# rizar/attention-lvcsr

Hardware: AMD Instinct MI355X
Metric: encoder+attention+decoder training frames/sec (whole node) (higher is better)
Workload: dtype f32; 1 GPU; wsj_base: B=16 utterances x T=800 frames x F=40 fbank per GPU, L=100 labels; 256x256x256x256 BiGRU subsample [1, 1, 2, 2], content_and_conv attention, 256-unit GRU decoder; global_batch=16, per_gpu_batch=16, ragged=False, parallelism=dp1, optimizer=clip100+adadelta+maxnorm1, hip_graph=True, priming_steps=2, encoder_kernels=persistent clusters, full=False

## Files before the change

attention-lvcsr_amd/csrc/gemm.hip:

```cpp
#include "common.h"
#include "lvsr_hip.h"
#include "graph_cache.h"

#define BM 64
#define BN 64
#define BK 16
#define LDS_LD (BM + 4)

struct GemmArgs {
    const float* A; const float* B; float* C; const float* bias;
    int M, N, K, lda, ldb, ldc, transA, transB;
    float alpha, beta;
    int ksplit;
    int kchunk;
    float* part;
    int batch;
    long long sA, sB, sC;
};

__global__ __launch_bounds__(256) void lvsr_sgemm_kernel(GemmArgs g) {
    __shared__ float As[BK][LDS_LD];
    __shared__ float Bs[BK][LDS_LD];
    const int tid = threadIdx.x, lane = tid & 63, wave = tid >> 6;
    const int m0 = blockIdx.y * BM, n0 = blockIdx.x * BN;
    int zsplit = blockIdx.z;
    if (g.batch > 1) {
        g.A += blockIdx.z * g.sA; g.B += blockIdx.z * g.sB; g.C += blockIdx.z * g.sC;
        zsplit = 0;
    }
    const int kbeg = zsplit * g.kchunk;
    const int kend = min(g.K, kbeg + g.kchunk);
    const int rowbase = (wave >> 1) * 32, colbase = (wave & 1) * 32;
    f32x4 acc[2][2];
#pragma unroll
    for (int i = 0; i < 2; ++i)
#pragma unroll
        for (int j = 0; j < 2; ++j) acc[i][j] = (f32x4){0.f, 0.f, 0.f, 0.f};

    for (int k0 = kbeg; k0 < kend; k0 += BK) {
        if (!g.transA) {
            const int kk = tid & 15, mm = tid >> 4;
#pragma unroll
            for (int p = 0; p < 4; ++p) {
                const int m = m0 + mm + p * 16, k = k0 + kk;
                As[kk][mm + p * 16] = (m < g.M && k < kend) ? g.A[(size_t)m * g.lda + k] : 0.f;
            }
        } else {
            const int mm = tid & 63, kk = tid >> 6;
#pragma unroll
            for (int p = 0; p < 4; ++p) {
                const int m = m0 + mm, k = k0 + kk + p * 4;
                As[kk + p * 4][mm] = (m < g.M && k < kend) ? g.A[(size_t)k * g.lda + m] : 0.f;
            }
        }
        if (!g.transB) {
            const int nn = tid & 63, kk = tid >> 6;
#pragma unroll
            for (int p = 0; p < 4; ++p) {
                const int n = n0 + nn, k = k0 + kk + p * 4;
                Bs[kk + p * 4][nn] = (n < g.N && k < kend) ? g.B[(size_t)k * g.ldb + n] : 0.f;
            }
        } else {
            const int kk = tid & 15, nn = tid >> 4;
#pragma unroll
            for (int p = 0; p < 4; ++p) {
                const int n = n0 + nn + p * 16, k = k0 + kk;
                Bs[kk][nn + p * 16] = (n < g.N && k < kend) ? g.B[(size_t)n * g.ldb + k] : 0.f;
            }
        }
        __syncthreads();
#pragma unroll
        for (int ks = 0; ks < BK; ks += 4) {
            const int kr = ks + (lane >> 4), li = lane & 15;
            float a[2], b[2];
            a[0] = As[kr][rowbase + li];
            a[1] = As[kr][rowbase + 16 + li];
            b[0] = Bs[kr][colbase + li];
            b[1] = Bs[kr][colbase + 16 + li];
#pragma unroll
            for (int i = 0; i < 2; ++i)
#pragma unroll
                for (int j = 0; j < 2; ++j)
                    acc[i][j] = __builtin_amdgcn_mfma_f32_16x16x4f32(a[i], b[j], acc[i][j], 0, 0, 0);
        }
        __syncthreads();
// ... 254 lines not shown
        if (more) {
            if (inside && k0 + 2 * GK <= kend) {
                gemm1_tile_load_fast<!TA, TM>(g.A, g.lda, m0, k0 + GK, ra);
                gemm1_tile_load_fast<TB, TN>(g.B, g.ldb, n0, k0 + GK, rb);
            } else {
                gemm1_tile_load<!TA, TM>(g.A, g.lda, m0, g.M, k0 + GK, kend, vecA, ra);
                gemm1_tile_load<TB, TN>(g.B, g.ldb, n0, g.N, k0 + GK, kend, vecB, rb);
            }
        }
        const int kr0 = lane >> 5, li = lane & 31;
        float pa[2][MI], pb[2][NI];
#pragma unroll
        for (int i = 0; i < MI; ++i) pa[0][i] = As[cur][kr0][wm + 32 * i + li];
#pragma unroll
        for (int j = 0; j < NI; ++j) pb[0][j] = Bs[cur][kr0][wn + 32 * j + li];
#pragma unroll
        for (int s = 0; s < GK / 2; ++s) {
            const int c = s & 1, n = c ^ 1;
            if (s + 1 < GK / 2) {
                const int kr = 2 * (s + 1) + kr0;
#pragma unroll
                for (int i = 0; i < MI; ++i) pa[n][i] = As[cur][kr][wm + 32 * i + li];
#pragma unroll
                for (int j = 0; j < NI; ++j) pb[n][j] = Bs[cur][kr][wn + 32 * j + li];
            }
            __builtin_amdgcn_sched_barrier(0);
#pragma unroll
            for (int i = 0; i < MI; ++i)
#pragma unroll
                for (int j = 0; j < NI; ++j)
                    acc[i][j] = __builtin_amdgcn_mfma_f32_32x32x2f32(pa[c][i], pb[c][j], acc[i][j], 0, 0, 0);
            __builtin_amdgcn_sched_barrier(0);
        }
        if (more) {
            gemm1_tile_store<!TA, TM>(As[cur ^ 1], ra);
            gemm1_tile_store<TB, TN>(Bs[cur ^ 1], rb);
        }
        __syncthreads();
        cur ^= 1;
    }
#pragma unroll
    for (int i = 0; i < MI; ++i)
#pragma unroll
        for (int j = 0; j < NI; ++j)
#pragma unroll
            for (int r = 0; r < 16; ++r) {
                const int m = m0 + wm + i * 32 + (r & 3) + 8 * (r >> 2) + 4 * (lane >> 5);
                const int n = n0 + wn + j * 32 + (lane & 31);
                if (m < g.M && n < g.N) {
                    if (g.ksplit > 1) {
                        g.part[((size_t)bz * g.M + m) * g.N + n] = acc[i][j][r];
                    } else {
                        float v = g.alpha * acc[i][j][r];
                        if (g.beta != 0.f) v += g.beta * g.C[(size_t)m * g.ldc + n];
                        if (g.bias) v += g.bias[n];
                        g.C[(size_t)m * g.ldc + n] = v;
                    }
                }
            }
}
template <bool TA, bool TB, bool FAST>
__device__ __forceinline__ void sgemm128_tile(GemmArgs g, int bx, int by, int bz) { sgemm_tile<128, 128, TA, TB, FAST>(g, bx, by, bz); }

template <bool TA, bool TB, bool FAST>
__global__ __launch_bounds__(256) void lvsr_sgemm64_kernel(GemmArgs g) {
    const int total = gridDim.x * gridDim.y * gridDim.z;
    const int t = gemm_xcd_order(blockIdx.x + gridDim.x * (blockIdx.y + gridDim.y * blockIdx.z), total);
    sgemm_tile_kmajor<64, 64, TA, TB, FAST>(g, t % gridDim.x, (t / gridDim.x) % gridDim.y, t / (gridDim.x * gridDim.y));
}

template <bool TA, bool TB, bool FAST>
__global__ __launch_bounds__(256) void lvsr_sgemm128_kernel(GemmArgs g) {
    const int total = gridDim.x * gridDim.y * gridDim.z;
    const int t = gemm_xcd_order(blockIdx.x + gridDim.x * (blockIdx.y + gridDim.y * blockIdx.z), total);
    sgemm128_tile<TA, TB, FAST>(g, t % gridDim.x, (t / gridDim.x) % gridDim.y, t / (gridDim.x * gridDim.y));
}

#define GROUP_MAX 40
struct GroupDesc {
    const float* A; const float* B; float* C;
    int M, N, K, lda, ldb, ldc;
    float beta;
    int ksplit, kchunk, gx, gy, unit0;
    long long part_off;
};
struct GroupPack { GroupDesc d[GROUP_MAX]; int n, total; float* part; };

template <bool FAST>
__global__ __launch_bounds__(256) void lvsr_sgemm128_grouped_tn_kernel(GroupPack pk) {
    const int t = gemm_xcd_order(blockIdx.x, pk.total);
    int p = 0;
    for (int x = 1; x < pk.n; ++x)
        if (t >= pk.d[x].unit0) p = x;
    const GroupDesc& d = pk.d[p];
    const int local = t - d.unit0;
    GemmArgs g;
    g.A = d.A; g.B = d.B; g.C = d.C; g.bias = nullptr;
    g.M = d.M; g.N = d.N; g.K = d.K; g.lda = d.lda; g.ldb = d.ldb; g.ldc = d.ldc; g.transA = 1; g.transB = 0;
    g.alpha = 1.f; g.beta = d.beta; g.ksplit = d.ksplit; g.kchunk = d.kchunk; g.part = pk.part + d.part_off;
    g.batch = 1; g.sA = g.sB = g.sC = 0;
    sgemm128_tile<true, false, FAST>(g, local % d.gx, (local / d.gx) % d.gy, local / (d.gx * d.gy));
}

__global__ __launch_bounds__(256) void lvsr_sgemm_grouped_reduce(GroupPack pk) {
    const GroupDesc& d = pk.d[blockIdx.y];
    if (d.ksplit <= 1) return;
    const size_t total = (size_t)d.M * d.N;
    const float* part = pk.part + d.part_off;
    for (size_t idx = (size_t)blockIdx.x * 256 + threadIdx.x; idx < total; idx += (size_t)gridDim.x * 256) {
        const int m = (int)(idx / d.N), n = (int)(idx % d.N);
        float s = 0.f;
        for (int z = 0; z < d.ksplit; ++z) s += part[(size_t)z * total + idx];
        if (d.beta != 0.f) s += d.beta * d.C[(size_t)m * d.ldc + n];
        d.C[(size_t)m * d.ldc + n] = s;
    }
}

__global__ __launch_bounds__(256) void lvsr_sgemm_splitk_reduce(GemmArgs g) {
    const size_t total = (size_t)g.M * g.N;
    for (size_t idx = (size_t)blockIdx.x * blockDim.x + threadIdx.x; idx < total; idx += (size_t)gridDim.x * blockDim.x) {
        const int m = (int)(idx / g.N), n = (int)(idx % g.N);
        float s = 0.f;
        for (int z = 0; z < g.ksplit; ++z) s += g.part[(size_t)z * total + idx];
        float v = g.alpha * s;
        if (g.beta != 0.f) v += g.beta * g.C[(size_t)m * g.ldc + n];
        if (g.bias) v += g.bias[n];
        g.C[(size_t)m * g.ldc + n] = v;
    }
}

__global__ __launch_bounds__(256) void lvsr_colsum_kernel(const float* X, int M, int N, int ldx, float* out, float beta,
                                                          int rows_per, float* part) {
    __shared__ float red[4][64];
    const int n = blockIdx.x * 64 + (threadIdx.x & 63);
    const int g = threadIdx.x >> 6;
    const int m0 = blockIdx.y * rows_per, m1 = min(M, m0 + rows_per);
    float s0 = 0.f, s1 = 0.f, s2 = 0.f, s3 = 0.f;
    if (n < N) {
        int m = m0 + g;
        for (; m + 12 < m1; m += 16) {
            s0 += X[(size_t)m * ldx + n];
            s1 += X[(size_t)(m + 4) * ldx + n];
            s2 += X[(size_t)(m + 8) * ldx + n];
            s3 += X[(size_t)(m + 12) * ldx + n];
        }
        for (; m < m1; m += 4) s0 += X[(size_t)m * ldx + n];
    }
    red[g][threadIdx.x & 63] = (s0 + s1) + (s2 + s3);
    __syncthreads();
    if (g == 0 && n < N) {
        const int c = threadIdx.x & 63;
        const float v = ((red[0][c] + red[1][c]) + red[2][c]) + red[3][c];
        if (part) part[(size_t)blockIdx.y * N + n] = v;
        else out[n] = (beta != 0.f ? beta * out[n] : 0.f) + v;
    }
}

#define COLSUM_MANY_MAX 32
struct ColsumMember { const float* X; float* out; float* part; int M, N, ldx, S, rows_per, nx, block0, fin0; float beta; };
struct ColsumPack { ColsumMember m[COLSUM_MANY_MAX]; int n; };
__global__ __launch_bounds__(256) void lvsr_colsum_many_kernel(ColsumPack pk) {
    __shared__ float red[4][64];
    int p = 0;
    for (int i = 1; i < pk.n; ++i)
        if ((int)blockIdx.x >= pk.m[i].block0) p = i;
    const ColsumMember& c = pk.m[p];
    const int local = blockIdx.x - c.block0, bx = local % c.nx, by = local / c.nx;
    const int n = bx * 64 + (threadIdx.x & 63);
    const int g = threadIdx.x >> 6;
    const int m0 = by * c.rows_per, m1 = min(c.M, m0 + c.rows_per);
    const float* X = c.X;
    const int ldx = c.ldx;
    float s0 = 0.f, s1 = 0.f, s2 = 0.f, s3 = 0.f;
    if (n < c.N) {
        int m = m0 + g;
        for (; m + 12 < m1; m += 16) {
            s0 += X[(size_t)m * ldx + n];
            s1 += X[(size_t)(m + 4) * ldx + n];
            s2 += X[(size_t)(m + 8) * ldx + n];
            s3 += X[(size_t)(m + 12) * ldx + n];
        }
        for (; m < m1; m += 4) s0 += X[(size_t)m * ldx + n];
    }
    red[g][threadIdx.x & 63] = (s0 + s1) + (s2 + s3);
    __syncthreads();
    if (g == 0 && n < c.N) {
        const int col = threadIdx.x & 63;
        const float v = ((red[0][col] + red[1][col]) + red[2][col]) + red[3][col];
        if (c.S > 1) c.part[(size_t)by * c.N + n] = v;
        else c.out[n] = (c.beta != 0.f ? c.beta * c.out[n] : 0.f) + v;
    }
}
__global__ __launch_bounds__(256) void lvsr_colsum_many_finish(ColsumPack pk) {
    int p = 0;
    for (int i = 1; i < pk.n; ++i)
        if ((int)blockIdx.x >= pk.m[i].fin0) p = i;
    const ColsumMember& c = pk.m[p];
// ... 73 lines not shown
    if (M == 0 || N == 0) return LVSR_OK;
    GemmArgs g;
    g.batch = batch; g.sA = sA; g.sB = sB; g.sC = sC;
    if (batch > 1) ws = nullptr;
    g.A = A; g.B = B; g.C = C; g.bias = bias;
    g.M = M; g.N = N; g.K = K; g.lda = lda; g.ldb = ldb; g.ldc = ldc; g.transA = transA; g.transB = transB;
    g.alpha = alpha; g.beta = beta; g.ksplit = 1; g.kchunk = 0; g.part = nullptr;
    const bool big = (M >= 96 && N >= 96) || (min(M, N) >= 32 && max(M, N) >= 256 && K >= 2048);
    int tm = big ? GM : BM, tn = big ? GN : BN;
    const int tk = big ? GK : BK;
    int tiles = ((M + tm - 1) / tm) * ((N + tn - 1) / tn);
    const int mid_max = lvsr_knob(LVSR_KNOB_GEMM_MID_TILES) > 0 ? lvsr_knob(LVSR_KNOB_GEMM_MID_TILES) : 2048;
    const bool mid = big && batch == 1 && (tiles < 256 || (tiles < mid_max && K <= 2048));
    if (mid) { tm = 64; tn = 64; tiles = ((M + 63) / 64) * ((N + 63) / 64); }
    g.kchunk = ((K + tk - 1) / tk) * tk;
    if (g.kchunk == 0) g.kchunk = tk;
    const int slots = mid ? 1024 : 512;
    if (ws && 2 * tiles <= slots && K >= 1024) {
        int want = (slots + tiles - 1) / tiles;
        int maxk = K / 256;
        if (want > maxk) want = maxk;
        long long need = (long long)want * M * N * 4;
        while (want > 1 && need > ws_bytes) { --want; need = (long long)want * M * N * 4; }
        if (want > 1) {
            int chunk = (K + want - 1) / want;
            chunk = ((chunk + tk - 1) / tk) * tk;
            g.ksplit = (K + chunk - 1) / chunk;
            g.kchunk = chunk;
            g.part = ws;
        }
    }
    dim3 grid((N + tn - 1) / tn, (M + tm - 1) / tm, batch > 1 ? batch : g.ksplit);
    hipStream_t st = (hipStream_t)stream;
    if (!big) {
        hipLaunchKernelGGL(lvsr_sgemm_kernel, grid, dim3(256), 0, st, g);
    } else {
        const bool fast = (lda & 3) == 0 && (ldb & 3) == 0 && (((size_t)A) & 15) == 0 && (((size_t)B) & 15) == 0 &&
                          (batch == 1 || ((sA & 3) == 0 && (sB & 3) == 0));
#define LVSR_GEMM128(TA_, TB_)                                                                              \
    do {                                                                                                    \
        if (fast) hipLaunchKernelGGL((lvsr_sgemm128_kernel<TA_, TB_, true>), grid, dim3(256), 0, st, g);    \
        else hipLaunchKernelGGL((lvsr_sgemm128_kernel<TA_, TB_, false>), grid, dim3(256), 0, st, g);        \
    } while (0)
#define LVSR_GEMM64(TA_, TB_)                                                                               \
    do {                                                                                                    \
        if (fast) hipLaunchKernelGGL((lvsr_sgemm64_kernel<TA_, TB_, true>), grid, dim3(256), 0, st, g);     \
        else hipLaunchKernelGGL((lvsr_sgemm64_kernel<TA_, TB_, false>), grid, dim3(256), 0, st, g);         \
    } while (0)
        if (mid) {
            if (!transA && !transB) LVSR_GEMM64(false, false);
            else if (transA && !transB) LVSR_GEMM64(true, false);
            else if (!transA && transB) LVSR_GEMM64(false, true);
            else LVSR_GEMM64(true, true);
        } else if (!transA && !transB) LVSR_GEMM128(false, false);
        else if (transA && !transB) LVSR_GEMM128(true, false);
        else if (!transA && transB) LVSR_GEMM128(false, true);
        else LVSR_GEMM128(true, true);
#undef LVSR_GEMM128
#undef LVSR_GEMM64
    }
    if (g.ksplit > 1) {
        int nb = (int)(((size_t)M * N + 255) / 256);
        if (nb > 2048) nb = 2048;
        hipLaunchKernelGGL(lvsr_sgemm_splitk_reduce, dim3(nb), dim3(256), 0, st, g);
    }
    return lvsr_check_launch("lvsr_sgemm");
}

int lvsr_sgemm(void* stream, int transA, int transB, int M, int N, int K, float alpha, const float* A, int lda,
               const float* B, int ldb, float beta, float* C, int ldc, const float* bias, float* ws,
               long long ws_bytes) {
    return sgemm_launch(stream, transA, transB, M, N, K, alpha, A, lda, B, ldb, beta, C, ldc, bias, ws, ws_bytes, 1, 0, 0, 0);
}

int lvsr_sgemm_batched(void* stream, int transA, int transB, int M, int N, int K, float alpha, const float* A, int lda,
                       long long strideA, const float* B, int ldb, long long strideB, float beta, float* C, int ldc,
                       long long strideC, int batch) {
    LVSR_REQUIRE(batch >= 0, "lvsr_sgemm_batched: negative batch");
    if (batch == 0) return LVSR_OK;
    return sgemm_launch(stream, transA, transB, M, N, K, alpha, A, lda, B, ldb, beta, C, ldc, nullptr, nullptr, 0, batch,
                        strideA, strideB, strideC);
}

int lvsr_sgemm_tn_grouped(void* stream, const lvsr_gemm_desc* descs, int n, float* ws, long long ws_bytes) {
    LVSR_REQUIRE(n >= 0 && (n == 0 || descs), "lvsr_sgemm_tn_grouped: bad arguments");
    hipStream_t st = (hipStream_t)stream;
    for (int i = 0; i < n; ++i)
        LVSR_REQUIRE(descs[i].A && descs[i].B && descs[i].C && descs[i].M > 0 && descs[i].N > 0 && descs[i].K > 0,
                     "lvsr_sgemm_tn_grouped: bad descriptor %d", i);
    auto aligned = [](const lvsr_gemm_desc& s) {
        return (s.lda & 3) == 0 && (s.ldb & 3) == 0 && (((size_t)s.A) & 15) == 0 && (((size_t)s.B) & 15) == 0;
    };
    int target = 1024;
    if (ws) {
        for (;; target += 512) {
            long long need = 0;
            bool splits = false;
            for (int i = 0; i < n; ++i) {
                const int want = (descs[i].K + target - 1) / target;
                if (want > 1) { need += (long long)want * descs[i].M * descs[i].N; splits = true; }
            }
            if (!splits || need * 4 <= ws_bytes) break;
        }
    }
    long long off = 0;
    for (int pass = 0; pass < 2; ++pass) {
        GroupPack pk;
        pk.n = 0; pk.part = ws;
        int units = 0;
        bool any_split = false;
        auto launch = [&]() {
            if (pk.n == 0) return;
            pk.total = units;
            if (pass == 0) hipLaunchKernelGGL(lvsr_sgemm128_grouped_tn_kernel<true>, dim3(units), dim3(256), 0, st, pk);
            else hipLaunchKernelGGL(lvsr_sgemm128_grouped_tn_kernel<false>, dim3(units), dim3(256), 0, st, pk);
            if (any_split) hipLaunchKernelGGL(lvsr_sgemm_grouped_reduce, dim3(32, pk.n), dim3(256), 0, st, pk);
            pk.n = 0; units = 0; any_split = false;
        };
        for (int i = 0; i < n; ++i) {
            const lvsr_gemm_desc& s = descs[i];
            if (aligned(s) != (pass == 0)) continue;
            if (pk.n == GROUP_MAX) launch();
            GroupDesc& d = pk.d[pk.n++];
            d.A = s.A; d.B = s.B; d.C = s.C; d.M = s.M; d.N = s.N; d.K = s.K; d.lda = s.lda; d.ldb = s.ldb; d.ldc = s.ldc; d.beta = s.beta;
            d.gx = (s.N + GN - 1) / GN; d.gy = (s.M + GM - 1) / GM;
            int want = ws ? (s.K + target - 1) / target : 1;
            int chunk = (s.K + want - 1) / want;
            chunk = ((chunk + GK - 1) / GK) * GK;
            d.kchunk = chunk;
            d.ksplit = (s.K + chunk - 1) / chunk;
            d.part_off = off;
            if (d.ksplit > 1) { off += (long long)d.ksplit * s.M * s.N; any_split = true; }
            d.unit0 = units;
            units += d.gx * d.gy * d.ksplit;
        }
        launch();
    }
    return lvsr_check_launch("lvsr_sgemm_tn_grouped");
}

int lvsr_colsum(void* stream, const float* X, int M, int N, int ldx, float* out, float beta, float* ws,
                long long ws_bytes) {
    if (N <= 0) return LVSR_OK;
    const int nx = (N + 63) / 64;
    int S = 1;
    if (ws && M >= 512) {
        S = (M + 255) / 256;
        const int want = (1024 + nx - 1) / nx;
        if (S > want) S = want;
        while (S > 1 && (long long)S * N * 4 > ws_bytes) --S;
    }
    const int rows_per = (M + S - 1) / S;
    hipLaunchKernelGGL(lvsr_colsum_kernel, dim3(nx, S), dim3(256), 0, (hipStream_t)stream, X, M, N, ldx, out, beta, rows_per,
                       S > 1 ? ws : nullptr);
    if (S > 1)
        hipLaunchKernelGGL(lvsr_colsum_finish, dim3((N + 255) / 256), dim3(256), 0, (hipStream_t)stream, ws, S, N, out, beta);
    return lvsr_check_launch("lvsr_colsum");
}

int lvsr_colsum_many(void* stream, const lvsr_colsum_desc* descs, int n, float* ws, long long ws_bytes, long long split_ws_bytes) {
    LVSR_REQUIRE(n >= 0 && (n == 0 || descs), "lvsr_colsum_many: bad arguments");
    for (int i = 0; i < n; ++i)
        LVSR_REQUIRE(descs[i].X && descs[i].out && descs[i].M >= 0 && descs[i].N > 0, "lvsr_colsum_many: bad descriptor %d", i);
    for (int i0 = 0; i0 < n; i0 += COLSUM_MANY_MAX) {
        ColsumPack pk;
        pk.n = n - i0 < COLSUM_MANY_MAX ? n - i0 : COLSUM_MANY_MAX;
        int blocks = 0, fin = 0;
        long long off = 0;
        bool any_split = false;
        for (int i = 0; i < pk.n; ++i) {
            const lvsr_colsum_desc& d = descs[i0 + i];
            ColsumMember& c = pk.m[i];
            c.X = d.X; c.out = d.out; c.M = d.M; c.N = d.N; c.ldx = d.ldx; c.beta = d.beta;
            c.nx = (d.N + 63) / 64;
            int S = 1;
            if (ws && d.M >= 512) {
                S = (d.M + 255) / 256;
                const int want = (1024 + c.nx - 1) / c.nx;
                if (S > want) S = want;
                while (S > 1 && (long long)S * d.N * 4 > split_ws_bytes) --S;
            }
            c.S = S;
            c.rows_per = (d.M + S - 1) / S;
            c.part = ws ? ws + off : nullptr;
            if (S > 1) { off += (long long)S * d.N; any_split = true; }
            c.block0 = blocks; blocks += c.nx * S;
            c.fin0 = fin; fin += (d.N + 255) / 256;
        }
        LVSR_REQUIRE(off * 4 <= ws_bytes, "lvsr_colsum_many: workspace too small for the partial sums (%lld bytes needed)", off * 4);
        if (blocks > 0) hipLaunchKernelGGL(lvsr_colsum_many_kernel, dim3(blocks), dim3(256), 0, (hipStream_t)stream, pk);
        if (any_split) hipLaunchKernelGGL(lvsr_colsum_many_finish, dim3(fin), dim3(256), 0, (hipStream_t)stream, pk);
        LVSR_REQUIRE(i0 + COLSUM_MANY_MAX >= n || !any_split, "lvsr_colsum_many: more than %d members with row splits", COLSUM_MANY_MAX);
    }
    return lvsr_check_launch("lvsr_colsum_many");
}

int lvsr_copy2d_many(void* stream, const lvsr_copy_desc* descs, int n) {
    LVSR_REQUIRE(n >= 0 && (n == 0 || descs), "lvsr_copy2d_many: bad arguments");
    for (int i = 0; i < n; ++i)
        LVSR_REQUIRE(descs[i].rows >= 0 && descs[i].cols >= 0 && descs[i].src && descs[i].dst, "lvsr_copy2d_many: bad descriptor %d", i);
    for (int i0 = 0; i0 < n; i0 += COPY_MANY_MAX) {
        CopyPack pk;
        pk.n = n - i0 < COPY_MANY_MAX ? n - i0 : COPY_MANY_MAX;
        for (int i = 0; i < pk.n; ++i) pk.d[i] = descs[i0 + i];
        hipLaunchKernelGGL(lvsr_copy2d_many_kernel, dim3(128, pk.n), dim3(256), 0, (hipStream_t)stream, pk);
    }
    return lvsr_check_launch("lvsr_copy2d_many");
}

int lvsr_transpose(void* stream, const float* in, int rows, int cols, float* out) {
    if (rows <= 0 || cols <= 0) return LVSR_OK;
    hipLaunchKernelGGL(lvsr_transpose_kernel, dim3((cols + 31) / 32, (rows + 31) / 32), dim3(256), 0, (hipStream_t)stream,
                       in, rows, cols, out);
    return lvsr_check_launch("lvsr_transpose");
// ... 41 lines not shown
```

attention-lvcsr_amd/lvsr_amd/bricks/__init__.py:

```python
import contextlib

import torch


class SpeechBottom(object):
    ACT = {"identity": 0, "rectifier": 2, "tanh": 3}

    def __init__(self, dims, store, lib, workspace):
        self.d, self.store, self.lib, self.ws = dims, store, lib, workspace
        self._saved = None

    def apply(self, recordings, save_for_backward=True):
        d, p, lib, ws = self.d, self.store.p, self.lib, self.ws
        if not d.bottom_dims:
            return recordings
        T, B = int(recordings.shape[0]), int(recordings.shape[1])
        x = recordings.contiguous().view(T * B, d.F)
        saved = []
        for j, o in enumerate(d.bottom_dims):
            z = ws.get("bottom%d.z" % j, (T * B, o))
            lib.sgemm(x, p["/recognizer/bottom/bottom/linear_%d.W" % j], z, bias=p["/recognizer/bottom/bottom/linear_%d.b" % j])
            a = ws.get("bottom%d.a" % j, (T * B, o))
            lib.call("lvsr_act_fwd", lib.stream_for(a), self.ACT[d.bottom_act], native_ptr(z), o, T * B, o, native_ptr(a), o)
            saved.append((x, z))
# ... 258 lines not shown
            x2, xg2 = x.view(T * B, I), xg.view(T * B, 6 * H)
            sync = self._sync_ws(i, B, H)
            pk = self._packed(i) if sync is None else None
            Wcat, bcat = self._fork_cat(i)
            lib.sgemm(x2, Wcat, xg2, bias=bcat)
            h0s = [p[self._names(i, direction)["h0"]] for direction in ("forward", "backward")]
            if sync is not None:
                nf, nb = self._names(i, "forward"), self._names(i, "backward")
                Whh, Whg = [p[nf["Whh"]], p[nb["Whh"]]], [p[nf["Whg"]], p[nb["Whg"]]]
            else:
                Whh, Whg = [pk["Whh"][0], pk["Whh"][1]], [pk["Whg"][0], pk["Whg"][1]]
            lib.run("lvsr_bigru_fwd", "lvsr_bigru_fwd_args", y, self.use_graph and sync is None, xg=xg, mask=m, Whh_p=Whh, Whg_p=Whg, h0=h0s,
                    y=y, ysub=(ysub if s > 1 else None), u=u, r=r, c=c, rh=rh, sub=s, T=T, B=B, H=H,
                    persistent=int(sync is not None), sync_ws=sync)
            saved.append(dict(x=x, mask=m, T=T, y=y, u=u, r=r, c=c, rh=rh))
            x = ysub
            if m is not None and s > 1:
                mm = ws.get(self._n(i, "msub"), (Ts, B))
                mm.copy_(m[::s])
                m = mm
            T = Ts
        if m is None:
            m = ws.get(self.pfx + ".ones_mask", (T, B))
            m.fill_(1.0)
        if save_for_backward:
            self._saved = saved
        return x, m

    def backward(self, d_encoded, need_input_grad=False):
        d, p, g, lib, ws = self.d, self.store.p, self.store.g, self.lib, self.ws
        if self._pass_cols is not None:
            return self._backward_in_passes(self._pass_cols, d_encoded, need_input_grad)
        assert self._saved is not None, "apply() must run first"
        gemm_ws = ws.get("gemm_ws", (1 << 22,))
        self._scatter = []
        dy = d_encoded.contiguous()
        B = int(dy.shape[1])
        for i in reversed(range(d.n_layers)):
            H, s, I = d.Hs[i], d.subsample[i], d.layer_input_dim(i)
            sv = self._saved[i]
            T = sv["T"]
            dxg = ws.get(self._n(i, "dxg"), (T, B, 6 * H))
            Bp = (B + 15) // 16 * 16
            dh_ws = ws.get(self._n(i, "dh"), (12 * Bp * H,))
            nf, nb = self._names(i, "forward"), self._names(i, "backward")
            sync = self._sync_ws(i, B, H)
            pk = self._packed(i) if sync is None else None
            if sync is not None:
                WhhT, WhgT = [p[nf["Whh"]], p[nb["Whh"]]], [p[nf["Whg"]], p[nb["Whg"]]]
            else:
                WhhT, WhgT = [pk["WhhT"][0], pk["WhhT"][1]], [pk["WhgT"][0], pk["WhgT"][1]]
            lib.run("lvsr_bigru_bwd", "lvsr_bigru_bwd_args", dxg, self.use_graph and sync is None, mask=sv["mask"], y=sv["y"],
                    u=sv["u"], r=sv["r"], c=sv["c"], WhhT_p=WhhT, WhgT_p=WhgT, h0=[p[nf["h0"]], p[nb["h0"]]], dy=dy,
                    dxg=dxg, dh_ws=dh_ws, dh0=[g[nf["h0"]], g[nb["h0"]]], sub=s, T=T, B=B, H=H,
                    persistent=int(sync is not None), sync_ws=sync)
            x2 = sv["x"].view(T * B, I)
            dxg2 = dxg.view(T * B, 6 * H)
            y2 = sv["y"].view(T * B, 2 * H)
            rh2 = sv["rh"].view(T * B, 2 * H)
            dx = None
            if i > 0 or need_input_grad:
                dx = ws.get(self._n(i, "dx"), (T, B, I))
            if dx is not None:
                lib.sgemm(dxg2, self._cats[i]["W"], dx.view(T * B, I), transB=True)
            with self._side_stream() as side_ws:
                for di, direction in enumerate(("forward", "backward")):
                    n = self._names(i, direction)
                    dc = dxg2[:, di * 3 * H: di * 3 * H + H]
                    dg = dxg2[:, di * 3 * H + H: di * 3 * H + 3 * H]
                    hcol = slice(di * H, (di + 1) * H)
                    lib.sgemm(rh2[:, hcol], dc, g[n["Whh"]], transA=True, ws=side_ws, group=True)
                    if T > 1:
                        if di == 0:
                            lib.sgemm(y2[: (T - 1) * B, hcol], dg[B:], g[n["Whg"]], transA=True, ws=side_ws, group=True)
                        else:
                            lib.sgemm(y2[B:, hcol], dg[: (T - 1) * B], g[n["Whg"]], transA=True, ws=side_ws, group=True)
                        beta = 1.0
                    else:
                        beta = 0.0
                    first = dg[:B] if di == 0 else dg[(T - 1) * B:]
                    lib.sgemm(p[n["h0"]], first, g[n["Whg"]], transA=True, beta=beta, M=H, K=B, lda=0, group=True)
                gW = ws.get("enc%d.gWcat" % i, (I, 6 * H))
                gb = ws.get("enc%d.gbcat" % i, (6 * H,))
                lib.sgemm(x2, dxg2, gW, transA=True, ws=side_ws)
                lib.colsum(dxg2, gb, ws=side_ws)
                for di, direction in enumerate(("forward", "backward")):
                    n = self._names(i, direction)
                    o = di * 3 * H
                    self._scatter += [(gW[:, o: o + H], g[n["Wi"]]), (gW[:, o + H: o + 3 * H], g[n["Wg"]]),
                                      (gb[o: o + H], g[n["bi"]]), (gb[o + H: o + 3 * H], g[n["bg"]])]
                if self.overlap and getattr(lib, "_group", None) is not None:
                    lib.flush_group(ws.get("gemm_ws.grouped.side", (1 << 26,)))
                    lib.begin_group()
            dy = dx
        self.join_side_stream()
        if getattr(lib, "_group", None) is None:
            self.finish_backward()
        return dy

    def finish_backward(self):
        self.lib.copy_many(self._scatter)
        self._scatter = []
```

include/lvsr_hip.h:

```cpp
#ifndef LVSR_HIP_H
#define LVSR_HIP_H

#ifdef __cplusplus
extern "C" {
#endif

const char* lvsr_last_error(void);
int lvsr_abi_version(void);
void lvsr_graph_clear(void);
int lvsr_graph_count(void);
void lvsr_graph_suppress(int on);
int lvsr_region_begin(void* stream, const char* key, long long key_bytes);
int lvsr_region_end(void* stream, int keep);
#define LVSR_KNOB_PERSIST_ROWS 0
#define LVSR_KNOB_PERSIST_FLAGS 1
#define LVSR_KNOB_PERSIST_THREADS 2
#define LVSR_KNOB_PHASE_CLOCK 3
#define LVSR_KNOB_MAX_CLUSTER_WGS 4
#define LVSR_KNOB_CLUSTER_RESERVE 5
#define LVSR_KNOB_GEMM_MID_TILES 6
#define LVSR_KNOB_DEC_CLUSTER 7
#define LVSR_KNOB_ENERGY_ROWS 8
#define LVSR_KNOB_COUNT 9
int lvsr_set_knob(int knob, int value);
int lvsr_get_knob(int knob);

int lvsr_sgemm(void* stream, int transA, int transB, int M, int N, int K, float alpha, const float* A, int lda,
               const float* B, int ldb, float beta, float* C, int ldc, const float* bias, float* ws,
               long long ws_bytes);
int lvsr_sgemm_batched(void* stream, int transA, int transB, int M, int N, int K, float alpha, const float* A, int lda,
                       long long strideA, const float* B, int ldb, long long strideB, float beta, float* C, int ldc,
                       long long strideC, int batch);
typedef struct lvsr_gemm_desc {
    const float* A; const float* B; float* C;
    int M, N, K, lda, ldb, ldc;
    float beta;
} lvsr_gemm_desc;
int lvsr_sgemm_tn_grouped(void* stream, const lvsr_gemm_desc* descs, int n, float* ws, long long ws_bytes);
typedef struct lvsr_copy_desc {
    const float* src; float* dst;
    int rows, cols, lds, ldd;
    float beta;
} lvsr_copy_desc;
int lvsr_copy2d_many(void* stream, const lvsr_copy_desc* descs, int n);
int lvsr_colsum(void* stream, const float* X, int M, int N, int ldx, float* out, float beta, float* ws,
                long long ws_bytes);
typedef struct lvsr_colsum_desc {
    const float* X; float* out;
    int M, N, ldx;
    float beta;
} lvsr_colsum_desc;
int lvsr_colsum_many(void* stream, const lvsr_colsum_desc* descs, int n, float* ws, long long ws_bytes, long long split_ws_bytes);
int lvsr_transpose(void* stream, const float* in, int rows, int cols, float* out);

long long lvsr_pack_size(int K, int N);
int lvsr_pack_b(void* stream, const float* W, int ldw, int K, int N, int trans, float* packed);
typedef struct lvsr_pack_desc {
    const float* W;
    float* packed;
    int ldw, K, N, trans;
} lvsr_pack_desc;
int lvsr_pack_b_many(void* stream, const lvsr_pack_desc* descs, int n, int use_graph);

typedef struct lvsr_bigru_fwd_args {
    const float* xg;
    const float* mask;
    const float* Whh_p[2];
    const float* Whg_p[2];
    const float* h0[2];
    float* y;
    float* ysub;
    float* u; float* r; float* c; float* rh;
    int sub, T, B, H;
    int kernel_mask;
    int persistent;
    void* sync_ws;
} lvsr_bigru_fwd_args;
int lvsr_bigru_fwd(void* stream, const lvsr_bigru_fwd_args* a, int use_graph);

typedef struct lvsr_bigru_bwd_args {
    const float* mask; const float* y; const float* u; const float* r; const float* c;
    const float* WhhT_p[2];
    const float* WhgT_p[2];
    const float* h0[2];
    const float* dy;
    float* dxg;
    float* dh_ws;
    float* dh0[2];
    int sub, T, B, H;
    int kernel_mask;
    int persistent;
    void* sync_ws;
} lvsr_bigru_bwd_args;
int lvsr_bigru_bwd(void* stream, const lvsr_bigru_bwd_args* a, int use_graph);
int lvsr_bigru_persist_rows(int B, int H);
long long lvsr_bigru_persist_ws_bytes(int B, int H);

typedef struct lvsr_attdec_args {
    int Tp, B, L, E, D, M, K, c;
    int prior_type;
    int step0;
    int phases;
    int normalizer;
    double p0, p1, p2, p3;
    const float* A; const float* PA; const float* Am;
    long long A_ts, A_bs, PA_ts, PA_bs, Am_ts, Am_bs;
    const float* Ws_p;
    const float* w_e;
    const float* e_bias;
    const float* filters;
    const float* handler;
    const float* Whg_p;
    const float* Whh_p;
    const float* Wdi_p;
    const float* Wdg_p;
    const float* xg;
    const float* ymask;
    float* S;
    float* W;
    float* pos;
    float* WA;
// ... 226 lines not shown
```

Baseline: 1.033 million frames/s.

## Balance grouped TN weight-gradient GEMMs with cost-model split-K planning and round ordering

Replaces the fixed split-K target in the grouped TN GEMM with a planner. The planner searches split depths against a round-based cost model that uses the device's occupancy-derived slot count, then sorts groups by depth and launches them with a round-robin block order across XCDs. The per-group reduction becomes a vectorized float4 fold kernel. The encoder input-weight gradient GEMM now joins the grouped batch when I>=128, so more weight-gradient work can share one balanced launch, at the cost of more host-side planning per call, which is mostly hidden by graph capture.

```diff
diff --git a/attention-lvcsr_amd/csrc/gemm.hip b/attention-lvcsr_amd/csrc/gemm.hip
--- a/attention-lvcsr_amd/csrc/gemm.hip
+++ b/attention-lvcsr_amd/csrc/gemm.hip
@@ -1,6 +1,7 @@
 #include "common.h"
 #include "lvsr_hip.h"
 #include "graph_cache.h"
+#include <vector>
 
 #define BM 64
 #define BN 64
@@ -421,13 +422,21 @@
     int M, N, K, lda, ldb, ldc;
     float beta;
     int ksplit, kchunk, gx, gy, unit0;
+    int fold0;
     long long part_off;
 };
-struct GroupPack { GroupDesc d[GROUP_MAX]; int n, total; float* part; };
+struct GroupPack { GroupDesc d[GROUP_MAX]; int n, total, cyc; float* part; };
+
+__device__ __forceinline__ int gemm_round_order(int L, int total, int G) {
+    const int round = 8 * G, full = total / round * round;
+    if (L >= full) return full + gemm_xcd_order(L - full, total - full);
+    const int l = L % round;
+    return L - l + (l & 7) * G + (l >> 3);
+}
 
 template <bool FAST>
 __global__ __launch_bounds__(256) void lvsr_sgemm128_grouped_tn_kernel(GroupPack pk) {
-    const int t = gemm_xcd_order(blockIdx.x, pk.total);
+    const int t = pk.cyc > 0 ? gemm_round_order(blockIdx.x, pk.total, pk.cyc) : gemm_xcd_order(blockIdx.x, pk.total);
     int p = 0;
     for (int x = 1; x < pk.n; ++x)
         if (t >= pk.d[x].unit0) p = x;
@@ -452,6 +461,48 @@
         for (int z = 0; z < d.ksplit; ++z) s += part[(size_t)z * total + idx];
         if (d.beta != 0.f) s += d.beta * d.C[(size_t)m * d.ldc + n];
         d.C[(size_t)m * d.ldc + n] = s;
+    }
+}
+
+__global__ __launch_bounds__(256) void lvsr_sgemm_grouped_fold(GroupPack pk) {
+    int p = 0;
+    for (int x = 1; x < pk.n; ++x)
+        if ((int)blockIdx.x >= pk.d[x].fold0) p = x;
+    const GroupDesc& d = pk.d[p];
+    const size_t total = (size_t)d.M * d.N;
+    const size_t i0 = ((size_t)((int)blockIdx.x - d.fold0) * 256 + threadIdx.x) * 4;
+    if (d.ksplit <= 1 || i0 >= total) return;
+    const float* part = pk.part + d.part_off + i0;
+    const bool vec = ((d.N | d.ldc) & 3) == 0 && (d.part_off & 3) == 0 && ((((size_t)pk.part) | ((size_t)d.C)) & 15) == 0;
+    if (vec) {
+        float4 s = make_float4(0.f, 0.f, 0.f, 0.f);
+        int z = 0;
+        for (; z + 4 <= d.ksplit; z += 4) {
+            const float4 v0 = *(const float4*)(part + (size_t)z * total), v1 = *(const float4*)(part + (size_t)(z + 1) * total);
+            const float4 v2 = *(const float4*)(part + (size_t)(z + 2) * total), v3 = *(const float4*)(part + (size_t)(z + 3) * total);
+            s.x += v0.x; s.y += v0.y; s.z += v0.z; s.w += v0.w;
+            s.x += v1.x; s.y += v1.y; s.z += v1.z; s.w += v1.w;
+            s.x += v2.x; s.y += v2.y; s.z += v2.z; s.w += v2.w;
+            s.x += v3.x; s.y += v3.y; s.z += v3.z; s.w += v3.w;
+        }
+        for (; z < d.ksplit; ++z) {
+            const float4 v = *(const float4*)(part + (size_t)z * total);
+            s.x += v.x; s.y += v.y; s.z += v.z; s.w += v.w;
+        }
+        float* c = d.C + (i0 / d.N) * (size_t)d.ldc + (i0 % d.N);
+        if (d.beta != 0.f) {
+            const float4 o = *(const float4*)c;
+            s.x += d.beta * o.x; s.y += d.beta * o.y; s.z += d.beta * o.z; s.w += d.beta * o.w;
+        }
+        *(float4*)c = s;
+    } else {
+        for (size_t idx = i0; idx < i0 + 4 && idx < total; ++idx) {
+            float s = 0.f;
+            for (int z = 0; z < d.ksplit; ++z) s += part[(size_t)z * total + (idx - i0)];
+            float* c = d.C + (idx / d.N) * (size_t)d.ldc + (idx % d.N);
+            if (d.beta != 0.f) s += d.beta * *c;
+            *c = s;
+        }
     }
 }
 
@@ -691,15 +742,170 @@
                         strideA, strideB, strideC);
 }
 
+static bool group_aligned(const lvsr_gemm_desc& s) {
+    return (s.lda & 3) == 0 && (s.ldb & 3) == 0 && (((size_t)s.A) & 15) == 0 && (((size_t)s.B) & 15) == 0;
+}
+
+static int group_slots() {
+    static int cached = 0;
+    if (cached == 0) {
+        int occ = 0, dev = 0, cus = 0;
+        const bool ok = hipOccupancyMaxActiveBlocksPerMultiprocessor(&occ, lvsr_sgemm128_grouped_tn_kernel<true>, 256, 0) == hipSuccess &&
+                        hipGetDevice(&dev) == hipSuccess &&
+                        hipDeviceGetAttribute(&cus, hipDeviceAttributeMultiprocessorCount, dev) == hipSuccess;
+        if (!ok) (void)hipGetLastError();
+        const int v = ok ? occ * cus : 0;
+        cached = v >= 8 ? v / 8 * 8 : 8;
+    }
+    return cached;
+}
+
+#define GROUP_UNIT_COST 5
+#define GROUP_FOLD_COST 5
+#define GROUP_MIN_DEPTH 8
+struct GroupBatch { int idx[GROUP_MAX]; int n; };
+
+static long long group_cost(const int* kt, const int* tiles, const long long* mn, int n, int D, int slots, int* dep, int* order,
+                            long long* need, int* rounds) {
+    *need = 0;
+    for (int i = 0; i < n; ++i) {
+        const int s = (kt[i] + D - 1) / D;
+        dep[i] = (kt[i] + s - 1) / s;
+        if (s > 1) *need += (long long)((kt[i] + dep[i] - 1) / dep[i]) * mn[i] + 3;
+        order[i] = i;
+    }
+    for (int i = 1; i < n; ++i)
+        for (int j = i; j > 0 && dep[order[j]] > dep[order[j - 1]]; --j) { const int t = order[j]; order[j] = order[j - 1]; order[j - 1] = t; }
+    long long cost = 0, cum = 0, r = 0, folded = 0;
+    for (int o = 0; o < n; ++o) {
+        const int i = order[o];
+        const int splits = (kt[i] + dep[i] - 1) / dep[i];
+        const long long units = (long long)tiles[i] * splits;
+        while (r * slots < cum + units) { cost += 2 * dep[i] + GROUP_UNIT_COST; ++r; }
+        cum += units;
+        if (splits > 1) folded += units;
+    }
+    *rounds = (int)r;
+    if (folded > 0) cost += GROUP_FOLD_COST + folded / 96;
+    return cost;
+}
+
+static long long group_plan_batch(const lvsr_gemm_desc* descs, const GroupBatch& b, bool split, long long avail, int slots, int launch,
+                                  long long off0, lvsr_gemm_plan* plan, int* units_out, int* rounds_out, int* depth_out) {
+    int kt[GROUP_MAX], tiles[GROUP_MAX], dep[GROUP_MAX], order[GROUP_MAX], maxkt = 1;
+    long long mn[GROUP_MAX];
+    for (int i = 0; i < b.n; ++i) {
+        const lvsr_gemm_desc& s = descs[b.idx[i]];
+        kt[i] = (s.K + GK - 1) / GK;
+        tiles[i] = ((s.N + GN - 1) / GN) * ((s.M + GM - 1) / GM);
+        mn[i] = (long long)s.M * s.N;
+        if (kt[i] > maxkt) maxkt = kt[i];
+    }
+    int best = maxkt, rounds = 0;
+    if (split) {
+        long long best_cost = -1, need;
+        const int step = maxkt > 4096 ? maxkt / 2048 : 1;
+        for (int D = maxkt; D >= GROUP_MIN_DEPTH; D -= step) {
+            const long long c = group_cost(kt, tiles, mn, b.n, D, slots, dep, order, &need, &rounds);
+            if (need <= avail && (best_cost < 0 || c < best_cost)) { best_cost = c; best = D; }
+        }
+    }
+    long long need;
+    group_cost(kt, tiles, mn, b.n, best, slots, dep, order, &need, &rounds);
+    long long off = off0;
+    int units = 0, deepest = 0;
+    for (int o = 0; o < b.n; ++o) {
+        const int i = order[o];
+        const lvsr_gemm_desc& s = descs[b.idx[i]];
+        lvsr_gemm_plan& q = plan[b.idx[i]];
+        q.launch = launch;
+        q.gx = (s.N + GN - 1) / GN; q.gy = (s.M + GM - 1) / GM;
+        q.kchunk = dep[i] * GK;
+        q.ksplit = (s.K + q.kchunk - 1) / q.kchunk;
+        q.part_off = 0;
+        if (q.ksplit > 1) { off = (off + 3) / 4 * 4; q.part_off = off; off += (long long)q.ksplit * s.M * s.N; }
+        q.unit0 = units;
+        units += q.gx * q.gy * q.ksplit;
+        if (q.kchunk > deepest) deepest = q.kchunk;
+    }
+    *units_out = units; *rounds_out = rounds; *depth_out = deepest;
+    return off - off0;
+}
+
+static int group_plan(const lvsr_gemm_desc* descs, int n, bool have_ws, long long ws_bytes, int slots, lvsr_gemm_plan* plan, int* summary) {
+    int launches = 0, units_all = 0, rounds_all = 0, deepest = 0;
+    long long off = 0;
+    const long long ws_floats = have_ws ? ws_bytes / 4 : 0;
+    for (int pass = 0; pass < 2; ++pass) {
+        GroupBatch b;
+        b.n = 0;
+        auto close = [&]() {
+            if (b.n == 0) return;
+            int units, rounds, depth;
+            off += group_plan_batch(descs, b, have_ws, ws_floats - off, slots, launches, off, plan, &units, &rounds, &depth);
+            ++launches; units_all += units; rounds_all += rounds;
+            if (depth > deepest) deepest = depth;
+            b.n = 0;
+        };
+        for (int i = 0; i < n; ++i) {
+            if (group_aligned(descs[i]) != (pass == 0)) continue;
+            if (b.n == GROUP_MAX) close();
+            b.idx[b.n++] = i;
+        }
+        close();
+    }
+    if (summary) { summary[0] = launches; summary[1] = units_all; summary[2] = rounds_all; summary[3] = deepest; }
+    return launches;
+}
+
+int lvsr_sgemm_tn_grouped_plan(const lvsr_gemm_desc* descs, int n, int have_ws, long long ws_bytes, int slots, lvsr_gemm_plan* plan,
+                               int* summary) {
+    LVSR_REQUIRE(n >= 0 && (n == 0 || (descs && plan)) && ws_bytes >= 0 && slots >= 0, "lvsr_sgemm_tn_grouped_plan: bad arguments");
+    for (int i = 0; i < n; ++i)
+        LVSR_REQUIRE(descs[i].M > 0 && descs[i].N > 0 && descs[i].K > 0, "lvsr_sgemm_tn_grouped_plan: bad descriptor %d", i);
+    group_plan(descs, n, have_ws != 0, ws_bytes, slots > 0 ? (slots >= 8 ? slots / 8 * 8 : 8) : group_slots(), plan, summary);
+    return LVSR_OK;
+}
+
+static int sgemm_tn_grouped_balanced(hipStream_t st, const lvsr_gemm_desc* descs, int n, float* ws, long long ws_bytes) {
+    if (n == 0) return LVSR_OK;
+    std::vector<lvsr_gemm_plan> plan((size_t)n);
+    const int slots = group_slots();
+    const int launches = group_plan(descs, n, ws != nullptr, ws_bytes, slots, plan.data(), nullptr);
+    for (int l = 0; l < launches; ++l) {
+        GroupPack pk;
+        pk.n = 0; pk.part = ws; pk.cyc = slots / 8; pk.total = 0;
+        int sel[GROUP_MAX];
+        for (int i = 0; i < n; ++i)
+            if (plan[i].launch == l) sel[pk.n++] = i;
+        for (int i = 1; i < pk.n; ++i)
+            for (int j = i; j > 0 && plan[sel[j]].unit0 < plan[sel[j - 1]].unit0; --j) { const int t = sel[j]; sel[j] = sel[j - 1]; sel[j - 1] = t; }
+        int fold = 0;
+        for (int o = 0; o < pk.n; ++o) {
+            const lvsr_gemm_desc& s = descs[sel[o]];
+            const lvsr_gemm_plan& q = plan[sel[o]];
+            GroupDesc& d = pk.d[o];
+            d.A = s.A; d.B = s.B; d.C = s.C; d.M = s.M; d.N = s.N; d.K = s.K; d.lda = s.lda; d.ldb = s.ldb; d.ldc = s.ldc; d.beta = s.beta;
+            d.gx = q.gx; d.gy = q.gy; d.kchunk = q.kchunk; d.ksplit = q.ksplit; d.unit0 = q.unit0; d.part_off = q.part_off;
+            d.fold0 = fold;
+            if (q.ksplit > 1) fold += (int)(((long long)s.M * s.N + 1023) / 1024);
+            pk.total += q.gx * q.gy * q.ksplit;
+        }
+        if (group_aligned(descs[sel[0]])) hipLaunchKernelGGL(lvsr_sgemm128_grouped_tn_kernel<true>, dim3(pk.total), dim3(256), 0, st, pk);
+        else hipLaunchKernelGGL(lvsr_sgemm128_grouped_tn_kernel<false>, dim3(pk.total), dim3(256), 0, st, pk);
+        if (fold > 0) hipLaunchKernelGGL(lvsr_sgemm_grouped_fold, dim3(fold), dim3(256), 0, st, pk);
+    }
+    return lvsr_check_launch("lvsr_sgemm_tn_grouped");
+}
+
 int lvsr_sgemm_tn_grouped(void* stream, const lvsr_gemm_desc* descs, int n, float* ws, long long ws_bytes) {
     LVSR_REQUIRE(n >= 0 && (n == 0 || descs), "lvsr_sgemm_tn_grouped: bad arguments");
     hipStream_t st = (hipStream_t)stream;
     for (int i = 0; i < n; ++i)
         LVSR_REQUIRE(descs[i].A && descs[i].B && descs[i].C && descs[i].M > 0 && descs[i].N > 0 && descs[i].K > 0,
                      "lvsr_sgemm_tn_grouped: bad descriptor %d", i);
-    auto aligned = [](const lvsr_gemm_desc& s) {
-        return (s.lda & 3) == 0 && (s.ldb & 3) == 0 && (((size_t)s.A) & 15) == 0 && (((size_t)s.B) & 15) == 0;
-    };
+    if (lvsr_knob(LVSR_KNOB_GEMM_GROUP_BALANCE) != 1) return sgemm_tn_grouped_balanced(st, descs, n, ws, ws_bytes);
+    auto aligned = group_aligned;
     int target = 1024;
     if (ws) {
         for (;; target += 512) {
@@ -715,7 +921,7 @@
     long long off = 0;
     for (int pass = 0; pass < 2; ++pass) {
         GroupPack pk;
-        pk.n = 0; pk.part = ws;
+        pk.n = 0; pk.part = ws; pk.cyc = 0;
         int units = 0;
         bool any_split = false;
         auto launch = [&]() {
@@ -738,7 +944,7 @@
             chunk = ((chunk + GK - 1) / GK) * GK;
             d.kchunk = chunk;
             d.ksplit = (s.K + chunk - 1) / chunk;
-            d.part_off = off;
+            d.part_off = off; d.fold0 = 0;
             if (d.ksplit > 1) { off += (long long)d.ksplit * s.M * s.N; any_split = true; }
             d.unit0 = units;
             units += d.gx * d.gy * d.ksplit;
diff --git a/attention-lvcsr_amd/lvsr_amd/bricks/__init__.py b/attention-lvcsr_amd/lvsr_amd/bricks/__init__.py
--- a/attention-lvcsr_amd/lvsr_amd/bricks/__init__.py
+++ b/attention-lvcsr_amd/lvsr_amd/bricks/__init__.py
@@ -364,7 +364,8 @@
                     lib.sgemm(p[n["h0"]], first, g[n["Whg"]], transA=True, beta=beta, M=H, K=B, lda=0, group=True)
                 gW = ws.get("enc%d.gWcat" % i, (I, 6 * H))
                 gb = ws.get("enc%d.gbcat" % i, (6 * H,))
-                lib.sgemm(x2, dxg2, gW, transA=True, ws=side_ws)
+                joins = I >= 128 and lib.get_knob("gemm_group_balance") != 1
+                lib.sgemm(x2, dxg2, gW, transA=True, ws=side_ws, group=joins)
                 lib.colsum(dxg2, gb, ws=side_ws)
                 for di, direction in enumerate(("forward", "backward")):
                     n = self._names(i, direction)
diff --git a/include/lvsr_hip.h b/include/lvsr_hip.h
--- a/include/lvsr_hip.h
+++ b/include/lvsr_hip.h
@@ -21,7 +21,8 @@
 #define LVSR_KNOB_GEMM_MID_TILES 6
 #define LVSR_KNOB_DEC_CLUSTER 7
 #define LVSR_KNOB_ENERGY_ROWS 8
-#define LVSR_KNOB_COUNT 9
+#define LVSR_KNOB_GEMM_GROUP_BALANCE 9
+#define LVSR_KNOB_COUNT 10
 int lvsr_set_knob(int knob, int value);
 int lvsr_get_knob(int knob);
 
@@ -37,6 +38,12 @@
     float beta;
 } lvsr_gemm_desc;
 int lvsr_sgemm_tn_grouped(void* stream, const lvsr_gemm_desc* descs, int n, float* ws, long long ws_bytes);
+typedef struct lvsr_gemm_plan {
+    int kchunk, ksplit, gx, gy, unit0, launch;
+    long long part_off;
+} lvsr_gemm_plan;
+int lvsr_sgemm_tn_grouped_plan(const lvsr_gemm_desc* descs, int n, int have_ws, long long ws_bytes, int slots, lvsr_gemm_plan* plan,
+                               int* summary);
 typedef struct lvsr_copy_desc {
     const float* src; float* dst;
     int rows, cols, lds, ldd;
```

Measured after the change: 1.053 million frames/s, median of 5. 1.9% higher.
